# bitlayer-org/tap-stark

Measured on AMD Instinct MI355X. Metric: trace cells/sec (proofs/sec alongside), 2^20x64 BabyBear trace, higher is better.
Workload: dtype u32

## Files before the change

tap-stark_amd/csrc/kernels.hpp:

```cpp
#pragma once
#include <stdint.h>

#include "bb.hpp"
#include "context.hpp"
#include "ntt_plan.hpp"

namespace ts {

struct ColMat {
    uint32_t* d = nullptr;
    uint64_t height = 0;
    uint32_t width = 0;
    uint64_t col_stride = 0;
};

void launch_build_twiddles(Context& ctx, uint32_t* W, uint32_t* Winv, unsigned log_size);
void launch_build_plant_twiddles(Context& ctx, uint2* WP, uint2* WPinv, unsigned log_size);
void launch_build_shift_tables(Context& ctx, uint32_t* lo, uint32_t* hi, uint32_t n_hi,
                               uint32_t n_cosets, uint32_t shift_mont, unsigned log_N,
                               unsigned log_blowup, uint32_t scale_mont);
const uint32_t* coset_scale_table(Context& ctx, unsigned log_n, unsigned log_blowup, uint32_t shift);
void launch_transpose_bitrev(Context& ctx, const uint32_t* src, uint32_t* dst, unsigned log_n,
                             uint32_t w, uint64_t dst_col_stride, uint32_t src_width = 0);
bool launch_transpose_bitrev_r16(Context& ctx, const uint32_t* src, uint32_t* dst, unsigned log_n, uint32_t w,
                                 uint64_t dst_col_stride, uint32_t src_width = 0);
void launch_transpose_plain(Context& ctx, const uint32_t* src, uint32_t* dst, uint64_t n, uint32_t w,
                            uint64_t dst_col_stride);
void launch_transpose_to_row_major(Context& ctx, const uint32_t* src, uint64_t col_stride,
                                   uint32_t* dst, uint64_t h, uint32_t w);
void launch_transpose_unbitrev(Context& ctx, const uint32_t* src, uint64_t col_stride, uint32_t* dst,
                               unsigned log_h, uint32_t w);
void coset_lde(Context& ctx, uint32_t* evals, uint64_t in_col_stride, uint32_t ncols, unsigned log_n,
               unsigned log_blowup, uint32_t shift, uint32_t* out, uint64_t out_col_stride,
               uint32_t beta0 = 0, uint32_t n_beta = 0, bool first_round_done = false,
               uint32_t* evals2 = nullptr, uint32_t shift2 = 0, uint32_t gw = 0, bool stage_timers = true);

constexpr uint32_t LDE_NO_OWN = 0xffffffffu;
int lde_own_coset_used(unsigned log_n, unsigned log_blowup, uint32_t shift);

inline void ntt_require_shape(const NttPlan& p, uint32_t ncols, uint64_t stride_a, uint64_t stride_b, bool lde) {
    if (const char* why = ntt_plan_refusal(p, ncols, stride_a, stride_b, lde)) throw Error(TS_ERR_INVALID, why);
}
void launch_contig_inverse(Context& ctx, const NttPlan& p, uint32_t* data, uint64_t col_stride, uint32_t ncols,
                           bool first_round_done = false, uint32_t* data2 = nullptr, uint32_t gw = 0xffffffffu);
void launch_contig_forward(Context& ctx, const NttPlan& p, uint32_t* data, uint64_t col_stride, uint32_t ncols,
                           uint32_t n_blocks, uint32_t gw = 0xffffffffu, uint32_t own_a = LDE_NO_OWN,
                           uint32_t own_b = LDE_NO_OWN);

void dft_columns(Context& ctx, uint32_t* cols, uint64_t col_stride, uint32_t ncols, unsigned log_n, bool inverse,
                 uint32_t shift);
void dft_batch(Context& ctx, const uint32_t* in, uint32_t* out, unsigned log_n, uint32_t w, bool inverse,
               uint32_t shift);
void coset_lde_batch(Context& ctx, const uint32_t* in, uint32_t* out, unsigned log_n, uint32_t w, unsigned added_bits,
                     uint32_t shift, bool bit_reversed);
void launch_bit_reverse_rows(Context& ctx, const uint32_t* src, uint32_t* dst, unsigned log_h, uint32_t w);

constexpr int MAX_BATCH_MATS = 64;
struct LeafMats {
    const uint32_t* d[MAX_BATCH_MATS];
    uint64_t col_stride[MAX_BATCH_MATS];
    uint32_t width[MAX_BATCH_MATS];
    uint8_t row_shift[MAX_BATCH_MATS];
    uint32_t n_mats;
    uint32_t total_width;
    const uint32_t* const* cols;
};
void launch_leaf_hash(Context& ctx, const LeafMats& mats, uint64_t height, uint32_t* digests);
void launch_leaf_hash_ef_pairs(Context& ctx, const uint32_t* vec, uint64_t n_rows, uint32_t* digests);
struct DevChallenger;
bool launch_merkle_levels(Context& ctx, uint32_t* tree, unsigned log_leaves,
                          DevChallenger* ch = nullptr, uint32_t* root_out = nullptr,
                          Ef* beta_out = nullptr);
void launch_merkle_tree_from(Context& ctx, uint32_t* tree, unsigned log_leaves, unsigned first_level,
                             DevChallenger* ch, uint32_t* root_out, Ef* beta_out);
bool leaf_tree_enabled(unsigned log_leaves);
void launch_commit_tree(Context& ctx, const LeafMats& mats, unsigned log_leaves, uint32_t* tree,
                        uint32_t* root_out = nullptr);
void launch_shard_top(Context& ctx, const uint32_t* subroots, uint32_t G, uint32_t* top,
                      DevChallenger* ch, uint32_t* root_out, Ef* beta_out);
void launch_merkle_one_level(Context& ctx, const uint32_t* children, uint32_t* parents,
                             uint64_t n_parents);
void launch_merkle_inject(Context& ctx, uint32_t* nodes, const uint32_t* inj, uint64_t n);
inline uint64_t merkle_level_offset(unsigned log_leaves, unsigned level) {
    uint64_t off = 0;
    for (unsigned l = 0; l < level; l++) off += (uint64_t)1 << (log_leaves - l);
    return off;
}
inline uint64_t merkle_total_digests(unsigned log_leaves) { return ((uint64_t)2 << log_leaves) - 1; }

struct AirProgram;
const uint32_t* selector_table(Context& ctx, unsigned log_n, unsigned log_qd, uint32_t shift);
constexpr int MAX_QUOTIENT_CHUNKS = 64;
struct QuotOut {
    uint32_t* chunk[MAX_QUOTIENT_CHUNKS];
};
constexpr uint32_t MAX_SIDE_MATS = 2;
struct SideLdes {
    uint32_t n = 0;
    const ColMat* m[MAX_SIDE_MATS] = {nullptr, nullptr};
};
void launch_quotient(Context& ctx, const AirProgram& air, const ColMat& trace_lde, unsigned log_n,
                     unsigned log_qd, const uint32_t* d_consts_mont, const uint32_t* d_alpha_pows_mont,
                     const QuotOut& out, uint64_t row_begin = 0, uint64_t row_end = 0,
                     uint32_t shift = GENERATOR, const SideLdes& side = SideLdes());
void launch_chunk_mix(Context& ctx, uint32_t* const* d_chunk_ptrs, uint32_t qd, uint64_t rows, uint64_t col_stride,
                      const uint32_t* d_mix_mont);

struct SideRows {
    uint32_t n = 0;
    const uint32_t* d[MAX_SIDE_MATS] = {nullptr, nullptr};
    uint32_t width[MAX_SIDE_MATS] = {0, 0};
};
void launch_check_constraints(Context& ctx, const AirProgram& air, const uint32_t* trace_row_major,
                              uint64_t n, const uint32_t* d_consts_mont,
                              unsigned long long* d_violation, const SideRows& side = SideRows());

void launch_bary_weights(Context& ctx, unsigned log_n, const Ef* points_mont, uint32_t n_points,
                         Ef* out, uint32_t coset_gen = 0);
struct BaryPending {
    DevBuf<uint32_t> partial[4];
    uint32_t* out[4] = {nullptr, nullptr, nullptr, nullptr};
    uint32_t n_blocks[4] = {0, 0, 0, 0}, n_words[4] = {0, 0, 0, 0};
    uint32_t n = 0, capacity = 2;
};
void launch_bary_dots(Context& ctx, const ColMat& m, unsigned log_n, const Ef* weights,
                      uint32_t n_points, Ef* out, BaryPending* pending = nullptr);
void launch_bary_finish(Context& ctx, BaryPending& pending);
struct ReduceArgs {
    Ef z_mont[2];
    Ef off_mont[2];
    Ef rys[2];
    uint32_t n_points;
    uint32_t accumulate;
};
void launch_reduce(Context& ctx, const ColMat& m, unsigned log_h, const uint32_t* d_alpha_pows_mont,
                   const ReduceArgs& args, Ef* ro);
struct FusedReduceArgs {
    Ef z_mont[2];
    Ef off_t[2];
    Ef k0, k1;
    const uint32_t* chunk_w;
    const uint32_t* chunk[MAX_QUOTIENT_CHUNKS];
    uint64_t chunk_stride;
    uint32_t n_chunks;
    uint64_t row0, rows;
};
struct LeadingMats {
    uint32_t n = 0;
    const ColMat* m[2] = {nullptr, nullptr};
    Ef off[2][2];
};
void launch_reduce_fused(Context& ctx, const ColMat& trace, unsigned log_h,
                         const uint32_t* d_alpha_pows_mont, const FusedReduceArgs& args, Ef* ro,
                         const LeadingMats& lead = LeadingMats());
void launch_reduce_low(Context& ctx, const ColMat& trace, unsigned log_n, const uint32_t* d_alpha_pows_mont,
                       const FusedReduceArgs& args, const Ef* weights, uint32_t* out);
void launch_ef_interleave(Context& ctx, const uint32_t* cols, uint64_t col_stride, uint64_t rows, Ef* out);

struct ClassJob {
    const uint32_t* d;
    uint64_t col_stride;
    uint32_t width;
    uint32_t has_next;
    const uint32_t* weights;
    Ef off[2];
};
struct ClassReduceArgs {
    Ef z_mont[2];
    Ef k0, k1;
};
void launch_reduce_class(Context& ctx, const ClassJob* d_jobs, uint32_t n_jobs, unsigned log_h,
                         const uint32_t* d_alpha_pows_mont, const ClassReduceArgs& args, Ef* ro);
struct BaryFinishJob {
    const uint32_t* partial;
    uint32_t* out;
    uint32_t n_blocks, n_words;
};
void launch_bary_finish_jobs(Context& ctx, const BaryFinishJob* d_jobs, const uint2* d_groups, uint32_t n_groups);

void launch_fri_fold(Context& ctx, const Ef* in, uint64_t h, Ef beta_canonical, Ef* out,
                     uint32_t* next_digests);
void launch_fri_fold_dev(Context& ctx, const Ef* in, uint64_t h, const Ef* d_beta, Ef* out,
                         uint32_t* next_digests, uint64_t h_global = 0, uint64_t row0 = 0);
struct FriRoundLaunch {
    const Ef* prev = nullptr;
    const Ef* d_beta_prev = nullptr;
    Ef* cur = nullptr;
    uint64_t h = 0;
    uint32_t* tree = nullptr;
    DevChallenger* ch = nullptr;
    uint32_t* root_out = nullptr;
    Ef* beta_out = nullptr;
    uint64_t h_global = 0, row0 = 0;
};
void launch_fri_commit_round(Context& ctx, const FriRoundLaunch& r);
constexpr int FRI_TAIL_LOG = 10;
constexpr uint32_t FRI_POW_NONE = 0xffffffffu;
void launch_fri_tail(Context& ctx, const Ef* in, uint32_t L0, uint32_t blowup, DevChallenger* ch,
                     Ef* tail_vecs, uint32_t* tail_trees, uint32_t* roots_out, Ef* betas_out,
                     Ef* final_out, uint32_t pow_bits = 0, uint32_t* pow_out = nullptr,
                     const Ef* beta_in = nullptr);
void launch_vec_add(Context& ctx, Ef* acc, const Ef* other, uint64_t n);
struct FriGatherDesc {
    const uint32_t* vec;
    const uint32_t* tree;
    uint32_t log_leaves;
    uint32_t shift;
    uint64_t out_vals;
    uint64_t out_path;
};
struct RowGatherJob {
    LeafMats mats;
    uint32_t shift;
    uint32_t pad;
    uint64_t out;
};
void launch_gather_queries(Context& ctx, const RowGatherJob* d_rows, uint32_t n_rows, uint32_t max_row_width,
                           const FriGatherDesc* d_descs, uint32_t n_descs, uint32_t max_log_leaves,
                           const uint32_t* d_indices, uint32_t n_idx, uint32_t* out);

double alu_ceiling(Context& ctx, int kind);
double bench_stage(Context& ctx, int stage, unsigned log_n, uint32_t width, unsigned log_blowup, uint32_t reps);

void launch_trace_fibonacci(Context& ctx, uint32_t* out, uint32_t a, uint32_t b, uint64_t n);
void launch_trace_synth_mul(Context& ctx, uint32_t* out, uint64_t n, uint32_t width, uint64_t seed);
void launch_trace_synth_ext(Context& ctx, uint32_t* out, uint64_t n, uint32_t width, uint64_t seed);

enum : uint8_t { COL_U32 = 0, COL_U16 = 1, COL_U8 = 2, COL_MONTY32 = 3, COL_MONTY31 = 4 };
struct IngestPlan {
    bool planar = false;
    uint64_t height = 0;
    uint32_t width = 0;
    uint64_t stride = 0;
    uint64_t bytes = 0;
    int uniform4 = -1;
    std::vector<uint64_t> table;
};
IngestPlan ingest_plan(const uint8_t* kinds, uint32_t n_kinds, bool planar, uint64_t row_stride, uint64_t height,
                       uint32_t width);
void launch_ingest(Context& ctx, const IngestPlan& plan, const uint8_t* src, uint32_t* out);
void launch_scale_words(Context& ctx, const uint32_t* in, uint32_t* out, uint64_t n, uint32_t mult);
uint32_t monty_ingest_factor(uint32_t kind);

}
```

tap-stark_amd/csrc/open.hip:

```cpp
#include "kernels.hpp"
#include "open_dev.hpp"

namespace ts {

constexpr int BW_ROWS = 4;

__global__ void __launch_bounds__(256)
k_bary_weights(unsigned log_n, const uint32_t* __restrict__ W, uint32_t gen_mont, Ef z0, Ef z1,
               uint32_t n_points, Ef* __restrict__ out) {
    const uint64_t n = 1ull << log_n;
    const uint64_t t0 = ((uint64_t)blockIdx.x * blockDim.x + threadIdx.x) * BW_ROWS;
    if (t0 >= n) return;
    Ef num[2 * BW_ROWS];
    uint32_t nrm[2 * BW_ROWS], pre[2 * BW_ROWS], xs[BW_ROWS];
    uint32_t run = R_MOD_P;
#pragma unroll
    for (int k = 0; k < BW_ROWS; k++) {
        const bool ok = t0 + k < n;
        uint32_t x = ok ? mont_mul(gen_mont, root_bitrev(W, log_n, t0 + k)) : R_MOD_P;
        xs[k] = x;
#pragma unroll
        for (int p = 0; p < 2; p++) {
            const Ef z = p == 0 ? z0 : z1;
            Ef u = Ef{{sub(z.c[0], x), z.c[1], z.c[2], z.c[3]}};
// ... 38 lines not shown
    constexpr int PER_THREAD = COLS * TR / 256;
    __shared__ uint32_t tile[16 * 257];
    __shared__ uint32_t wts[TR][NP * 4];
    __shared__ uint32_t red[4 * RS][COLS][NP * 4];
    const uint64_t n = 1ull << log_n;
    const uint32_t c0 = blockIdx.y * COLS;
    const uint32_t lane = threadIdx.x & 63, wv = threadIdx.x >> 6;
    const uint32_t cl = lane % COLS, rs = lane / COLS;
    const uint32_t sub = wv * RS + rs;
    const uint64_t row_begin = (uint64_t)blockIdx.x * rows_per_block;
    const uint64_t row_end = row_begin + rows_per_block < n ? row_begin + rows_per_block : n;
    uint64_t acc[NP * 4];
#pragma unroll
    for (int j = 0; j < NP * 4; j++) acc[j] = 0;
    for (uint64_t row0 = row_begin; row0 < row_end; row0 += TR) {
        uint32_t v[PER_THREAD];
#pragma unroll
        for (int k = 0; k < PER_THREAD; k++) {
            const uint32_t e = threadIdx.x + (uint32_t)k * 256;
            const uint32_t c = c0 + e / TR;
            const uint64_t t = row0 + e % TR;
            v[k] = (c < width && t < row_end) ? m[(uint64_t)c * col_stride + t] : 0u;
        }
        for (uint32_t e = threadIdx.x; e < (uint32_t)(TR * NP); e += 256) {
            const uint32_t p = e / TR, tt = e % TR;
            const uint64_t t = row0 + tt;
            Ef w = ef_zero();
            if (t < row_end) w = weights[(uint64_t)p * n + t];
            wts[tt][p * 4 + 0] = w.c[0];
            wts[tt][p * 4 + 1] = w.c[1];
            wts[tt][p * 4 + 2] = w.c[2];
            wts[tt][p * 4 + 3] = w.c[3];
        }
#pragma unroll
        for (int k = 0; k < PER_THREAD; k++) {
            const uint32_t e = threadIdx.x + (uint32_t)k * 256;
            const uint32_t t = e % TR;
            tile[(t & 15) * 257 + (t >> 4) * COLS + e / TR] = v[k];
        }
        __syncthreads();
#pragma unroll
        for (int rr = 0; rr < 16; rr++) {
            const uint32_t tt = sub * 16 + rr;
            const uint32_t x = tile[rr * 257 + sub * COLS + cl];
#pragma unroll
            for (int j = 0; j < NP * 4; j++) acc[j] = lazy_mac(acc[j], x, wts[tt][j]);
            if (rr & 1) {
#pragma unroll
                for (int j = 0; j < NP * 4; j++) acc[j] = lazy_fix(acc[j]);
            }
        }
        __syncthreads();
    }
#pragma unroll
    for (int j = 0; j < NP * 4; j++) red[sub][cl][j] = lazy_finish(acc[j]);
    __syncthreads();
    for (uint32_t idx = threadIdx.x; idx < (uint32_t)(COLS * NP * 4); idx += 256) {
        const uint32_t c = idx / (NP * 4), j = idx % (NP * 4);
        uint32_t sum = 0;
#pragma unroll
        for (int q = 0; q < 4 * RS; q++) sum = add(sum, red[q][c][j]);
        if (c0 + c < width)
            partial[((uint64_t)blockIdx.x * width + c0 + c) * (NP * 4) + j] = sum;
    }
}

template <int N>
struct BaryFinishArgs {
    BaryFinishJob j[N];
    uint32_t groups[N];
};
template <int N>
__global__ void __launch_bounds__(256)
k_bary_finish(BaryFinishArgs<N> a) {
    BaryFinishJob j = a.j[0];
    uint32_t group = blockIdx.x, first = 0;
#pragma unroll
    for (int k = 1; k < N; k++) {
        first += a.groups[k - 1];
        if (blockIdx.x >= first) {
            j = a.j[k];
            group = blockIdx.x - first;
        }
    }
    bary_finish_group(j.partial, j.out, j.n_blocks, j.n_words, group);
}

template <int N>
static void launch_bary_finish_n(Context& ctx, const char* name, const BaryPending& pend) {
    BaryFinishArgs<N> a{};
    uint32_t total = 0;
    for (uint32_t i = 0; i < pend.n; i++) {
        a.j[i] = BaryFinishJob{pend.partial[i].p, pend.out[i], pend.n_blocks[i], pend.n_words[i]};
        a.groups[i] = (pend.n_words[i] + 3) / 4;
        total += a.groups[i];
    }
    TS_LAUNCH_NAMED(ctx, name, k_bary_finish<N>, dim3(total), dim3(256), 0, a);
}

void launch_bary_finish(Context& ctx, BaryPending& pend) {
    if (pend.n == 0) return;
    if (pend.n == 4)
        launch_bary_finish_n<4>(ctx, "k_bary_finish<4>", pend);
    else if (pend.n == 3)
        launch_bary_finish_n<3>(ctx, "k_bary_finish<3>", pend);
    else
        launch_bary_finish_n<2>(ctx, "k_bary_finish<2>", pend);
    TS_HIP(hipGetLastError());
    for (uint32_t i = 0; i < pend.n; i++) pend.partial[i].reset();
    pend.n = 0;
}

void launch_bary_dots(Context& ctx, const ColMat& m, unsigned log_n, const Ef* weights,
                      uint32_t n_points, Ef* out, BaryPending* pending) {
    const uint64_t n = 1ull << log_n;
    const bool narrow = m.width <= 8;
    const uint32_t tr = narrow ? 512 : 64;
    uint32_t n_blocks = (uint32_t)((n + tr - 1) / tr);
    if (n_blocks > 2048) n_blocks = 2048;
    uint32_t rows_per_block = (uint32_t)(((n + n_blocks - 1) / n_blocks + tr - 1) / tr * tr);
    n_blocks = (uint32_t)((n + rows_per_block - 1) / rows_per_block);
    const uint32_t n_words = m.width * n_points * 4;
    DevBuf<uint32_t> partial(&ctx, (size_t)n_blocks * n_words);
    const uint32_t* md = m.d;
    if (narrow) {
        dim3 grid(n_blocks, (m.width + 7) / 8);
        if (n_points == 2)
            TS_LAUNCH(ctx, (k_bary_dots<2, 8>), grid, dim3(256), 0, md, m.col_stride, m.width, log_n,
                      weights, partial.p, rows_per_block);
        else
            TS_LAUNCH(ctx, (k_bary_dots<1, 8>), grid, dim3(256), 0, md, m.col_stride, m.width, log_n,
                      weights, partial.p, rows_per_block);
    } else {
        dim3 grid(n_blocks, (m.width + 63) / 64);
        if (n_points == 2)
            TS_LAUNCH(ctx, (k_bary_dots<2, 64>), grid, dim3(256), 0, md, m.col_stride, m.width, log_n,
                      weights, partial.p, rows_per_block);
        else
            TS_LAUNCH(ctx, (k_bary_dots<1, 64>), grid, dim3(256), 0, md, m.col_stride, m.width, log_n,
                      weights, partial.p, rows_per_block);
    }
    TS_HIP(hipGetLastError());
    BaryPending own;
    BaryPending& pend = pending ? *pending : own;
    if (pend.n == pend.capacity) launch_bary_finish(ctx, pend);
    pend.partial[pend.n] = std::move(partial);
    pend.out[pend.n] = reinterpret_cast<uint32_t*>(out);
    pend.n_blocks[pend.n] = n_blocks;
    pend.n_words[pend.n] = n_words;
    pend.n++;
    if (!pending) launch_bary_finish(ctx, pend);
}

template <int NP>
__global__ void __launch_bounds__(256)
k_reduce(const uint32_t* __restrict__ m, uint64_t col_stride, uint32_t width, unsigned log_h,
         const uint32_t* __restrict__ W, uint32_t gen_mont, const uint32_t* __restrict__ alpha_pows,
         ReduceArgs args, Ef* __restrict__ ro) {
    const uint64_t h = 1ull << log_h;
    const uint64_t X = (uint64_t)blockIdx.x * blockDim.x + threadIdx.x;
    if (X >= h) return;
    const Ef S = row_dot_alpha(m, col_stride, width, X, alpha_pows);
    const uint32_t x = mont_mul(gen_mont, root_bitrev(W, log_h, X));
    Ef inv_d[NP];
    inv_denoms<NP>(x, args.z_mont, inv_d);
    Ef acc = args.accumulate ? ro[X] : ef_zero();
#pragma unroll
    for (int p = 0; p < NP; p++) {
        Ef t = ef_mul(ef_sub(S, args.rys[p]), args.off_mont[p]);
        acc = ef_add(acc, ef_mul(t, inv_d[p]));
    }
    ro[X] = acc;
}

void launch_reduce(Context& ctx, const ColMat& m, unsigned log_h, const uint32_t* d_alpha_pows_mont,
                   const ReduceArgs& args, Ef* ro) {
    TS_REQUIRE(args.n_points >= 1 && args.n_points <= 2, TS_ERR_INVALID, "reduce: 1 or 2 points");
    ctx.ensure_twiddles(log_h == 0 ? 1 : log_h);
    const uint64_t h = 1ull << log_h;
    dim3 grid((unsigned)((h + 255) / 256));
    if (args.n_points == 2)
        TS_LAUNCH(ctx, k_reduce<2>, grid, dim3(256), 0, (const uint32_t*)m.d, m.col_stride, m.width,
                  log_h, (const uint32_t*)ctx.d_twiddle_fwd, to_mont(GENERATOR), d_alpha_pows_mont, args,
                  ro);
    else
        TS_LAUNCH(ctx, k_reduce<1>, grid, dim3(256), 0, (const uint32_t*)m.d, m.col_stride, m.width,
                  log_h, (const uint32_t*)ctx.d_twiddle_fwd, to_mont(GENERATOR), d_alpha_pows_mont, args,
                  ro);
    TS_HIP(hipGetLastError());
}

template <int EXTRA>
struct ExtraReduceArgs {
    struct {
        const uint32_t* d;
        uint64_t stride;
        uint32_t width;
        Ef off[2];
    } m[EXTRA ? EXTRA : 1];
};

template <int EXTRA, bool LOW>
__global__ void __launch_bounds__(256)
k_reduce_fused(const uint32_t* __restrict__ trace, uint64_t trace_stride, uint32_t width, unsigned log_h,
               const uint32_t* __restrict__ W, uint32_t gen_mont, const uint32_t* __restrict__ alpha_pows,
               FusedReduceArgs a, ExtraReduceArgs<EXTRA> e, const Ef* __restrict__ weights,
               uint32_t* __restrict__ out) {
    const uint64_t X = (uint64_t)blockIdx.x * blockDim.x + threadIdx.x;
    if (X >= a.rows) return;
    const Ef St = row_dot_alpha(trace, trace_stride, width, X, alpha_pows);
    Ef inv_d[2];
    if constexpr (!LOW) {
        const uint32_t x = mont_mul(gen_mont, root_bitrev(W, log_h, a.row0 + X));
        inv_denoms<2>(x, a.z_mont, inv_d);
    }
    uint64_t acc[4] = {0, 0, 0, 0};
    uint32_t c = 0;
    for (; c + 2 <= a.n_chunks; c += 2) {
        uint32_t v[8];
#pragma unroll
        for (int k = 0; k < 8; k++) v[k] = a.chunk[c + (k >> 2)][(uint64_t)(k & 3) * a.chunk_stride + X];
        const uint32_t* ap = a.chunk_w + 16 * c;
#pragma unroll
        for (int k = 0; k < 8; k++) {
#pragma unroll
            for (int j = 0; j < 4; j++) acc[j] = lazy_mac(acc[j], v[k], ap[4 * k + j]);
            if (k & 1) {
#pragma unroll
                for (int j = 0; j < 4; j++) acc[j] = lazy_fix(acc[j]);
            }
        }
    }
    for (; c < a.n_chunks; c++) row_dot_acc(acc, a.chunk[c], a.chunk_stride, 4, X, a.chunk_w + 16 * c);
    const Ef D{{lazy_finish(acc[0]), lazy_finish(acc[1]), lazy_finish(acc[2]), lazy_finish(acc[3])}};
    if constexpr (LOW) {
        const uint32_t nxi = neg(mont_mul(gen_mont, root_bitrev(W, log_h, X)));
        inv_d[0] = ef_mul_base(weights[X], nxi);
        inv_d[1] = ef_mul_base(weights[a.rows + X], nxi);
    }
    Ef g0 = ef_add(ef_mul(St, a.off_t[0]), D), g1 = ef_mul(St, a.off_t[1]);
#pragma unroll
    for (int i = 0; i < EXTRA; i++) {
        const Ef S = row_dot_alpha(e.m[i].d, e.m[i].stride, e.m[i].width, X, alpha_pows);
        g0 = ef_add(g0, ef_mul(S, e.m[i].off[0]));
        g1 = ef_add(g1, ef_mul(S, e.m[i].off[1]));
    }
    const Ef r = ef_add(ef_mul(ef_sub(g0, a.k0), inv_d[0]), ef_mul(ef_sub(g1, a.k1), inv_d[1]));
    if constexpr (LOW) {
#pragma unroll
        for (int k = 0; k < 4; k++) out[(uint64_t)k * a.rows + X] = r.c[k];
    } else {
        *reinterpret_cast<uint4*>(out + 4 * X) = make_uint4(r.c[0], r.c[1], r.c[2], r.c[3]);
    }
}

template <int EXTRA>
static void launch_reduce_fused_n(Context& ctx, const char* name, const ColMat& trace, unsigned log_h,
                                  const uint32_t* d_alpha_pows_mont, const FusedReduceArgs& a,
                                  const LeadingMats& lead, Ef* ro) {
    ExtraReduceArgs<EXTRA> e{};
    for (int i = 0; i < EXTRA; i++) {
        e.m[i].d = lead.m[i]->d;
        e.m[i].stride = lead.m[i]->col_stride;
        e.m[i].width = lead.m[i]->width;
        e.m[i].off[0] = lead.off[i][0];
        e.m[i].off[1] = lead.off[i][1];
    }
    TS_LAUNCH_NAMED(ctx, name, (k_reduce_fused<EXTRA, false>), dim3((unsigned)((a.rows + 255) / 256)), dim3(256), 0,
                    (const uint32_t*)trace.d, trace.col_stride, trace.width, log_h,
                    (const uint32_t*)ctx.d_twiddle_fwd, to_mont(GENERATOR), d_alpha_pows_mont, a, e,
                    (const Ef*)nullptr, reinterpret_cast<uint32_t*>(ro));
}

void launch_reduce_fused(Context& ctx, const ColMat& trace, unsigned log_h,
                         const uint32_t* d_alpha_pows_mont, const FusedReduceArgs& args, Ef* ro,
                         const LeadingMats& lead) {
    TS_REQUIRE(args.n_chunks <= (uint32_t)MAX_QUOTIENT_CHUNKS, TS_ERR_INVALID, "reduce_fused: too many chunks");
    ctx.ensure_twiddles(log_h == 0 ? 1 : log_h);
    FusedReduceArgs a = args;
    if (a.rows == 0) {
        a.row0 = 0;
        a.rows = 1ull << log_h;
    }
    TS_REQUIRE(a.row0 + a.rows <= (1ull << log_h), TS_ERR_INVALID, "reduce_fused: row range");
    TS_REQUIRE(lead.n <= 2, TS_ERR_INVARIANT, "reduce_fused: more than two leading matrices");
    for (uint32_t i = 0; i < lead.n; i++) {
        const ColMat* m = lead.m[i];
        TS_REQUIRE(m && m->d && a.row0 == 0 && m->height == a.rows && m->col_stride >= a.rows, TS_ERR_INVALID,
                   "reduce_fused: preprocessed or aux matrix shape");
    }
    if (lead.n == 2)
        launch_reduce_fused_n<2>(ctx, "k_reduce_fused_pre_aux", trace, log_h, d_alpha_pows_mont, a, lead, ro);
    else if (lead.n == 1)
        launch_reduce_fused_n<1>(ctx, "k_reduce_fused_pre", trace, log_h, d_alpha_pows_mont, a, lead, ro);
    else
        launch_reduce_fused_n<0>(ctx, "k_reduce_fused", trace, log_h, d_alpha_pows_mont, a, lead, ro);
    TS_HIP(hipGetLastError());
}

void launch_reduce_low(Context& ctx, const ColMat& trace, unsigned log_n, const uint32_t* d_alpha_pows_mont,
                       const FusedReduceArgs& args, const Ef* weights, uint32_t* out) {
    TS_REQUIRE(args.n_chunks <= (uint32_t)MAX_QUOTIENT_CHUNKS, TS_ERR_INVALID, "reduce_low: too many chunks");
    const uint64_t n = 1ull << log_n;
    TS_REQUIRE(args.row0 == 0 && trace.height >= n && trace.col_stride >= n && args.chunk_stride >= n, TS_ERR_INVALID,
               "reduce_low: the matrices must start with the low coset");
    ctx.ensure_twiddles(log_n == 0 ? 1 : log_n);
// ... 24 lines not shown
```

tap-stark_amd/csrc/prover.cpp:

```cpp
#include <string.h>

#include <algorithm>

#include "logup.hpp"
#include "prover_internal.hpp"

namespace ts {

void mmcs_commit(Context& ctx, PcsData& data) {
    const unsigned log_H = data.log_height;
    const uint64_t N = 1ull << log_H;
    bool uniform = true;
    for (auto& cm : data.ldes) uniform = uniform && cm.height == N;
    {
        StageTimer t(&ctx, "merkle_commit");
        data.tree = DevBuf<uint32_t>(&ctx, merkle_total_digests(log_H) * 8);
        std::vector<const uint32_t*> cols;
        struct Group { uint64_t height; size_t first; uint32_t total; };
        std::vector<Group> groups;
        for (unsigned lh = log_H + 1; lh-- > 0;) {
            const std::vector<const uint32_t*> gc = column_pointers(data.ldes, 1ull << lh);
            if (!gc.empty()) groups.push_back(Group{1ull << lh, cols.size(), (uint32_t)gc.size()});
            cols.insert(cols.end(), gc.begin(), gc.end());
        }
// ... 28 lines not shown
            DevBuf<uint32_t> inj(&ctx, 8 * (N / 2));
            size_t gi = 1;
            for (unsigned l = 1; l <= log_H; l++) {
                uint32_t* children = data.tree.p + 8 * merkle_level_offset(log_H, l - 1);
                uint32_t* parents = data.tree.p + 8 * merkle_level_offset(log_H, l);
                const uint64_t n_par = N >> l;
                launch_merkle_one_level(ctx, children, parents, n_par);
                if (gi < groups.size() && groups[gi].height == n_par) {
                    group_leaves(groups[gi], inj.p);
                    launch_merkle_inject(ctx, parents, inj.p, n_par);
                    gi++;
                }
            }
        }
        if (mail) {
            ctx.sync_point(mail, 32);
            memcpy(data.root, mail, 32);
        } else {
            d2h_sync(ctx, data.root, data.tree.p + 8 * (merkle_total_digests(log_H) - 1), 32);
        }
    }
}

std::unique_ptr<PcsData> TwoAdicFriPcs::commit(std::vector<DeviceMatrix>& evals,
                                               const std::vector<uint32_t>& domain_shifts, bool build_tree,
                                               bool keep_row_major) {
    auto data = std::make_unique<PcsData>();
    lde_stage(ctx_, fri_, evals, domain_shifts, 0, 0, true, *data, keep_row_major);
    if (build_tree) mmcs_commit(ctx_, *data);
    return data;
}

void check_side_matrix(const PcsData& data, const AirProgram& air, uint32_t i, uint64_t lde_height) {
    const bool aux = air.side_is_aux(i);
    const std::string what = aux ? "aux data" : "preprocessed key";
    TS_REQUIRE(data.ldes.size() == 1, TS_ERR_INVALID, what + ": exactly one committed matrix expected");
    TS_REQUIRE(i < air.n_side() && data.ldes[0].width == air.side_width(i), TS_ERR_INVALID,
               what + ": width differs from the AIR's " + (aux ? "aux" : "preprocessed") + " width");
    TS_REQUIRE(data.ldes[0].height == lde_height, TS_ERR_INVALID,
               what + ": LDE height is not the trace height << log_blowup");
}

std::vector<DeviceMatrix> TwoAdicFriPcs::quotient_chunks(const PcsData& trace_data,
                                                         const AirProgram& air,
                                                         const std::vector<uint32_t>& pis, Ef alpha,
                                                         const SideData& side) {
    TS_REQUIRE(trace_data.ldes.size() >= 1, TS_ERR_INVALID, "quotient: no trace matrix");
    TS_REQUIRE(trace_data.log_height >= fri_.log_blowup, TS_ERR_INVALID, "quotient: bad trace data");
    TS_REQUIRE(side.size() <= MAX_SIDE_MATS, TS_ERR_INVALID, "quotient: more than two committed side matrices");
    SideLdes ldes;
    for (const PcsData* d : side) {
        check_side_matrix(*d, air, ldes.n, trace_data.ldes[0].height);
        ldes.m[ldes.n++] = &d->ldes[0];
    }
    return quotient_chunks_slab(trace_data.ldes[0], trace_data.log_height - fri_.log_blowup, Slab{}, air,
                                pis, alpha, GENERATOR, ldes);
}

std::vector<DeviceMatrix> TwoAdicFriPcs::quotient_chunks_slab(const ColMat& lde_slab, unsigned log_n,
                                                              const Slab& slab, const AirProgram& air,
                                                              const std::vector<uint32_t>& pis, Ef alpha,
                                                              uint32_t domain_shift, const SideLdes& side) {
    StageTimer t(&ctx_, "compute quotient polynomial");
    TS_REQUIRE(side.n == air.n_side(), TS_ERR_INVALID,
               "quotient: an AIR needs the committed key of its preprocessed columns and the committed aux trace of "
               "its aux columns, and only such an AIR takes them");
    TS_REQUIRE(side.n == 0 || slab.rows == 0, TS_ERR_UNSUPPORTED, "quotient: preprocessed or aux columns on a slab");
    TS_REQUIRE(lde_slab.width == air.width, TS_ERR_INVALID, "quotient: trace width != AIR width");
    TS_REQUIRE(pis.size() == air.n_public_slots(), TS_ERR_INVALID, "quotient: wrong number of public values");
    const unsigned lqd = air.log_quotient_degree;
    TS_REQUIRE(lqd <= fri_.log_blowup, TS_ERR_INVARIANT,
               "quotient domain larger than the committed LDE (log_quotient_degree > log_blowup)");
    const uint64_t n = 1ull << log_n, qn = n << lqd;
    const uint32_t qd = 1u << lqd;
    const uint64_t slab_rows = slab.rows ? slab.rows : lde_slab.height;
    const uint64_t row_begin = std::min<uint64_t>(slab.row0, qn);
    const uint64_t row_end = std::min<uint64_t>(slab.row0 + slab_rows, qn);
    TS_REQUIRE(row_begin % n == 0 && row_end % n == 0, TS_ERR_INVALID, "quotient: slab must hold whole cosets");

    std::vector<uint32_t> consts = air_consts_mont(air, pis.data(), pis.size());
    consts.resize((consts.size() + 3) & ~(size_t)3, 0);
    const size_t n_consts = consts.size();
    const uint32_t K = air.n_constraints;
    const std::vector<uint32_t> pw = alpha_powers_mont(alpha, K);
    consts.resize(n_consts + std::max<size_t>(4 * (size_t)K, 4), 0);
    for (uint32_t i = 0; i < K; i++) memcpy(&consts[n_consts + 4 * (size_t)(K - 1 - i)], &pw[4 * (size_t)i], 16);
    DevBuf<uint32_t> d_consts(&ctx_, consts.size());
    h2d(ctx_, d_consts.p, consts.data(), consts.size() * 4);

    std::vector<DeviceMatrix> chunks(qd);
    QuotOut qo;
    memset(&qo, 0, sizeof qo);
    for (uint32_t c = 0; c < qd; c++) {
        chunks[c].buf = DevBuf<uint32_t>(&ctx_, 4 * n);
        chunks[c].height = n;
        chunks[c].width = 4;
        chunks[c].layout = DeviceMatrix::COL_MAJOR_BITREV;
        qo.chunk[c] = chunks[c].buf.p;
    }
    if (row_begin < row_end) {
        ColMat lde = lde_slab;
        lde.d = lde_slab.d - slab.row0;
        launch_quotient(ctx_, air, lde, log_n, lqd, d_consts.p, d_consts.p + n_consts, qo, row_begin, row_end,
                        domain_shift, side);
    }
    return chunks;
}

DevBuf<Ef> TwoAdicFriPcs::open_reduce(const PcsData& trace_data, const PcsData& quotient_data, Ef zeta,
                                      Ef alpha, std::vector<Ef>& opened_values, const SideData& side) {
    TS_REQUIRE(trace_data.log_height == quotient_data.log_height, TS_ERR_INVALID,
               "open: trace and quotient LDE heights differ");
    return open_reduce_slab(trace_data, quotient_data, trace_data.log_height, Slab{}, zeta, alpha,
                            opened_values, side);
}

DevBuf<Ef> TwoAdicFriPcs::open_reduce_slab(const PcsData& trace_data, const PcsData& quotient_data,
                                           unsigned log_N, const Slab& slab, Ef zeta, Ef alpha,
                                           std::vector<Ef>& opened_values, const SideData& side) {
    TS_REQUIRE(trace_data.ldes.size() == 1, TS_ERR_UNSUPPORTED, "open: one trace matrix expected");
    TS_REQUIRE(side.size() <= MAX_SIDE_MATS, TS_ERR_INVALID, "open: more than two rounds before the trace's");
    LeadingMats lead;
    for (const PcsData* d : side) {
        TS_REQUIRE(slab.rows == 0 && d->ldes.size() == 1 && d->ldes[0].height == trace_data.ldes[0].height,
                   TS_ERR_INVALID, "open: preprocessed or aux round shape");
        lead.m[lead.n++] = &d->ldes[0];
    }
    const unsigned log_n = log_N - fri_.log_blowup;
    const uint64_t n = 1ull << log_n;
    const uint64_t N = slab.rows ? slab.rows : 1ull << log_N;
    TS_REQUIRE(N >= n && trace_data.ldes[0].height == N, TS_ERR_INVALID, "open: slab shape");
    const uint32_t coset_gen =
        mul(GENERATOR, pow_canon(two_adic_generator(log_N), bitrev32(slab.beta0, fri_.log_blowup)));
    const ColMat& tr = trace_data.ldes[0];
    const uint32_t w = tr.width;
    const uint32_t qd = (uint32_t)quotient_data.ldes.size();
    for (auto& m : quotient_data.ldes)
        TS_REQUIRE(m.width == 4, TS_ERR_INVALID, "open: quotient chunks must have width 4");
    ctx_.ensure_twiddles(std::max(1u, log_N));
    const ColMat* two_point[3];
    uint32_t n_two = 0, max_w = 4;
    size_t chunks_at = 0;
    for (uint32_t i = 0; i < lead.n; i++) two_point[n_two++] = lead.m[i];
    two_point[n_two++] = &tr;
    for (uint32_t i = 0; i < n_two; i++) {
        chunks_at += 2 * (size_t)two_point[i]->width;
        max_w = std::max(max_w, two_point[i]->width);
    }

    const Ef zeta_next = efc_mul_base(zeta, two_adic_generator(log_n));
    const Ef pts_mont[2] = {ef_to_mont(zeta), ef_to_mont(zeta_next)};

    std::vector<Ef> raw(chunks_at + 4 * (size_t)qd);
    DevBuf<Ef> weights(&ctx_, 2 * n);
    {
        StageTimer t(&ctx_, "compute opened values with Lagrange interpolation");
        launch_bary_weights(ctx_, log_n, pts_mont, 2, weights.p, coset_gen);
        Ef* const mail = reinterpret_cast<Ef*>(ctx_.mailbox(4 * raw.size()));
        BaryPending pend;
        pend.capacity = n_two + 1;
        Ef* sums = mail;
        for (uint32_t i = 0; i < n_two; i++) {
            launch_bary_dots(ctx_, *two_point[i], log_n, weights.p, 2, sums, &pend);
            sums += 2 * (size_t)two_point[i]->width;
        }
        ColMat all;
        if (qd > 1 && columns_as_one_matrix(quotient_data.ldes, quotient_data.ldes[0].height, 0, all) &&
            all.width == 4 * qd) {
            launch_bary_dots(ctx_, all, log_n, weights.p, 1, sums, &pend);
        } else {
            for (uint32_t c = 0; c < qd; c++)
                launch_bary_dots(ctx_, quotient_data.ldes[c], log_n, weights.p, 1, sums + 4 * c, &pend);
        }
        launch_bary_finish(ctx_, pend);
        ctx_.sync_point(mail, raw.size() * sizeof(Ef));
        memcpy(raw.data(), mail, raw.size() * sizeof(Ef));
    }
    const Ef scale[2] = {bary_scale(zeta, coset_gen, n), bary_scale(zeta_next, coset_gen, n)};
    opened_values.assign(raw.size(), ef_zero());
    size_t at = 0;
    for (uint32_t i = 0; i < n_two; i++) {
        opened_from_raw(&raw[at], two_point[i]->width, 2, scale, &opened_values[at]);
        at += 2 * (size_t)two_point[i]->width;
    }
    opened_from_raw(&raw[at], 4 * qd, 1, scale, &opened_values[at]);

    StageTimer t(&ctx_, "reduce rows");
    const bool low = slab.rows == 0 && lead.n == 0 && reduce_low_wanted(w + 4 * qd);
    if (!low) weights.reset();
    DevBuf<Ef> ro(&ctx_, N);
    TS_REQUIRE(qd <= (uint32_t)MAX_QUOTIENT_CHUNKS, TS_ERR_UNSUPPORTED, "open: more than 64 quotient chunks");
    FusedReduceArgs a;
    memset(&a, 0, sizeof a);
    a.z_mont[0] = pts_mont[0];
    a.z_mont[1] = pts_mont[1];
    a.n_chunks = qd;
    a.chunk_stride = N;
    a.row0 = slab.row0;
    a.rows = N;
    AlphaLedger ledger(alpha, max_w);
    const Ef* ys = opened_values.data();
    for (uint32_t i = 0; i < n_two; i++) {
        const uint32_t mw = two_point[i]->width;
        Ef* const off = i < lead.n ? lead.off[i] : a.off_t;
        for (int p = 0; p < 2; p++, ys += mw) off[p] = ledger.visit(log_N, ys, mw, p).off;
    }
    std::vector<uint32_t> words = ledger.powers();
    const size_t n_apow = words.size();
    for (uint32_t c = 0; c < qd; c++, ys += 4) {
        TS_REQUIRE(quotient_data.ldes[c].col_stride == N, TS_ERR_INVALID, "open: chunk stride");
        a.chunk[c] = quotient_data.ldes[c].d;
        ledger.fold_weights(ledger.visit(log_N, ys, 4, 0).off, 4, words);
    }
    a.k0 = ledger.k(log_N, 0);
    a.k1 = ledger.k(log_N, 1);
    DevBuf<uint32_t> d_apow(&ctx_, words.size());
    h2d(ctx_, d_apow.p, words.data(), words.size() * 4);
    a.chunk_w = d_apow.p + n_apow;
    if (low) {
        DevBuf<uint32_t> ro_low(&ctx_, 4 * n), ro_cols(&ctx_, 4 * N);
        launch_reduce_low(ctx_, tr, log_n, d_apow.p, a, weights.p, ro_low.p);
        coset_lde(ctx_, ro_low.p, n, 4, log_n, fri_.log_blowup, 1, ro_cols.p, N, 0, 0, false, nullptr, 0, 0,
                  false);
        launch_ef_interleave(ctx_, ro_cols.p, N, N, ro.p);
    } else {
        launch_reduce_fused(ctx_, tr, log_N, d_apow.p, a, ro.p, lead);
    }
    return ro;
}

void TwoAdicFriPcs::open_batch(const PcsData& d, uint64_t index, std::vector<uint32_t>& rows,
                               std::vector<uint32_t>& path) {
    TS_REQUIRE(index < (1ull << d.log_height), TS_ERR_INVALID, "open_batch: index out of range");
    QueryGather qg(ctx_);
    const unsigned li = qg.add_indices({(uint32_t)index});
    const QueryGather::Slot o_rows = qg.add_rows(li, d.leaf_mats(), 0), o_path = qg.add_path(li, d.tree.p, d.log_height, 0);
    qg.run();
    rows.assign(qg.data(o_rows, 0), qg.data(o_rows, 0) + o_rows.words);
    path.assign(qg.data(o_path, 0), qg.data(o_path, 0) + o_path.words);
}

void TwoAdicFriPcs::fri_prove(std::vector<DevBuf<Ef>>& inputs, const std::vector<unsigned>& log_lens,
                              BfChallenger& challenger,
                              const std::vector<const PcsData*>& input_rounds,
                              std::vector<uint32_t>& pf, bool pass_through) {
    Context& ctx = ctx_;
    const FriConfig& fri = fri_;
    TS_REQUIRE(!inputs.empty() && inputs.size() == log_lens.size(), TS_ERR_INVALID, "FRI: no input");
    std::vector<const Ef*> in_ptr;
    for (auto& v : inputs) in_ptr.push_back(v.p);
    if (pass_through)
        TS_REQUIRE(input_rounds.empty() && log_lens.back() >= 1, TS_ERR_INVALID,
                   "FRI: pass-through input proof takes no committed batches");
    for (size_t k = 1; k < log_lens.size(); k++)
        TS_REQUIRE(log_lens[k] < log_lens[k - 1], TS_ERR_INVALID, "FRI: inputs must descend in height");
    const unsigned log_max_height = log_lens[0];
    TS_REQUIRE(log_lens.back() >= fri.log_blowup, TS_ERR_INVALID, "FRI: vector shorter than the blowup");
    for (const PcsData* d : input_rounds)
        TS_REQUIRE(d->log_height <= log_max_height, TS_ERR_INVALID,
                   "FRI: a committed batch is taller than every opened matrix");

    FriCommit st;
    Ef final_poly;
    {
        StageTimer t(&ctx, "FRI commit phase");
        fri_commit_begin(ctx, fri, log_max_height, challenger, st);
        fri_commit_rounds(ctx, fri, std::move(inputs[0]), 1ull << log_max_height, inputs, log_lens, 1, st);
        final_poly = fri_commit_finish(ctx, fri, challenger, st);
    }
    std::vector<FriRound>& rounds = st.rounds;
    const uint32_t R = (uint32_t)rounds.size();

    uint32_t pow_witness;
    {
        StageTimer t(&ctx, "grind for proof-of-work witness");
        pow_witness = fri_pow_witness(ctx, challenger, fri.proof_of_work_bits, st);
    }

    StageTimer tq(&ctx, "query phase");
    const uint32_t Q = fri.num_queries;
    std::vector<uint32_t> indices(Q);
    for (uint32_t q = 0; q < Q; q++) indices[q] = (uint32_t)challenger.sample_bits(log_max_height);

    const size_t n_in_rounds = input_rounds.size();
    QueryGather qg(ctx);
    const unsigned li = qg.add_indices(indices);
    std::vector<QueryGather::Slot> o_rows(n_in_rounds), o_path(n_in_rounds);
    for (size_t k = 0; k < n_in_rounds; k++) {
        const unsigned lh = input_rounds[k]->log_height;
        o_rows[k] = qg.add_rows(li, input_rounds[k]->leaf_mats(), log_max_height - lh);
        o_path[k] = qg.add_path(li, input_rounds[k]->tree.p, lh, log_max_height - lh);
    }
    std::vector<QueryGather::Opening> o_round(R);
    for (uint32_t r = 0; r < R; r++)
        o_round[r] = qg.add_round(li, rounds[r].vec, rounds[r].tree, rounds[r].log_leaves, r + 1);
    std::vector<QueryGather::Slot> o_pass(pass_through ? in_ptr.size() : 0);
    for (size_t k = 0; k < o_pass.size(); k++)
        o_pass[k] = qg.add_values(li, in_ptr[k], log_max_height - log_lens[k] + 1);
    qg.run();

    std::vector<ProofWriter::Batch> batches;
    for (const PcsData* d : input_rounds) batches.push_back({&d->ldes, d->log_height});
    std::vector<unsigned> round_depths;
    for (auto& r : rounds) round_depths.push_back(r.log_leaves);
    pf.reserve(pf.size() + 16 + 8 * (size_t)R +
               (size_t)Q * ProofWriter::words_per_query(batches, round_depths, o_pass.size()));
    ProofWriter pw(pf);
    pw.begin_rounds(R);
    for (uint32_t r = 0; r < R; r++) pw.commitment(rounds[r].root, 8);
    pw.begin_queries(Q);
    for (uint32_t q = 0; q < Q; q++) {
        pw.begin_input_proof((uint32_t)(pass_through ? in_ptr.size() : n_in_rounds));
        for (size_t k = 0; k < o_pass.size(); k++) {
            const uint32_t half = (indices[q] >> (log_max_height - log_lens[k])) & 1;
            pw.pass_through_value(log_lens[k], qg.data(o_pass[k], q) + 4 * half);
        }
        for (size_t k = 0; k < n_in_rounds; k++) {
            const unsigned lh = input_rounds[k]->log_height;
            pw.batch_opening(input_rounds[k]->ldes, qg.data(o_rows[k], q), lh, {{qg.data(o_path[k], q), lh}});
        }
        for (uint32_t r = 0; r < R; r++)
            pw.round_opening(qg.data(o_round[r].vals, q), rounds[r].log_leaves,
                             {{qg.data(o_round[r].path, q), rounds[r].log_leaves}});
    }
    pw.finish(final_poly, pow_witness);
}

std::vector<uint32_t> TwoAdicFriPcs::open(const std::vector<OpenRound>& rounds, BfChallenger& challenger,
                                          std::vector<Ef>& opened_values) {
    TS_REQUIRE(!rounds.empty(), TS_ERR_INVALID, "open: no rounds");
    const Ef alpha = challenger.sample();
    uint32_t max_w = 1;
    unsigned log_global_max = 0;
    for (auto& r : rounds) {
        TS_REQUIRE(r.data && r.points.size() == r.data->ldes.size(), TS_ERR_INVALID,
                   "open: one point list per committed matrix");
        for (auto& m : r.data->ldes) max_w = std::max(max_w, m.width);
        log_global_max = std::max(log_global_max, r.data->log_height);
    }
    ctx_.ensure_twiddles(std::max(1u, log_global_max));
    AlphaLedger ledger(alpha, max_w);
// ... 204 lines not shown
```

Before: 26.36 billion.

## Fuse barycentric weight computation with multi-matrix dot products in one kernel

Adds a kernel that computes the Lagrange barycentric weights for each row block into shared memory and immediately takes dot products against the trace and quotient-chunk matrices in the same launch. This avoids a separate weights kernel, writing and re-reading the weights array from global memory, and one launch per matrix. The weights buffer is now allocated and written only when the later low-reduce or lead matrices need it. In exchange, each block carries a larger shared-memory footprint and recomputes the inversions per block, and the lead matrices are still handled by the older path.

```diff
diff --git a/tap-stark_amd/csrc/kernels.hpp b/tap-stark_amd/csrc/kernels.hpp
--- a/tap-stark_amd/csrc/kernels.hpp
+++ b/tap-stark_amd/csrc/kernels.hpp
@@ -126,6 +126,14 @@
 void launch_bary_dots(Context& ctx, const ColMat& m, unsigned log_n, const Ef* weights,
                       uint32_t n_points, Ef* out, BaryPending* pending = nullptr);
 void launch_bary_finish(Context& ctx, BaryPending& pending);
+constexpr int BARY_LIST_MAX = 4;
+struct BaryListMat {
+    const ColMat* m;
+    uint32_t n_points;
+    Ef* out;
+};
+void launch_bary_dots_list(Context& ctx, const BaryListMat* mats, uint32_t n_mats, unsigned log_n,
+                           const Ef* points_mont, uint32_t coset_gen, Ef* weights_out, BaryPending& pending);
 struct ReduceArgs {
     Ef z_mont[2];
     Ef off_mont[2];
diff --git a/tap-stark_amd/csrc/open.hip b/tap-stark_amd/csrc/open.hip
--- a/tap-stark_amd/csrc/open.hip
+++ b/tap-stark_amd/csrc/open.hip
@@ -214,6 +214,182 @@
     if (!pending) launch_bary_finish(ctx, pend);
 }
 
+constexpr int BL_ROWS = 512;
+
+template <int NP, int COLS>
+__device__ __forceinline__ void bary_dots_group(const uint32_t* __restrict__ m, uint64_t col_stride, uint32_t width,
+                                                uint32_t c0, uint64_t row0, uint64_t row_end,
+                                                uint32_t (*wts)[BL_ROWS][4], uint32_t* tile,
+                                                uint32_t* __restrict__ partial, bool first) {
+    constexpr int RS = 64 / COLS;
+    constexpr int TR = 16 * 4 * RS;
+    constexpr int PER_THREAD = COLS * TR / 256;
+    static_assert(BL_ROWS % TR == 0 && 256 * NP * 4 <= 16 * 257, "image and tile shapes");
+    uint32_t tid = threadIdx.x;
+    asm volatile("" : "+v"(tid));
+    const uint32_t lane = tid & 63, wv = tid >> 6;
+    const uint32_t cl = lane % COLS, rs = lane / COLS;
+    const uint32_t sub = wv * RS + rs;
+    const uint64_t img_end = row0 + BL_ROWS < row_end ? row0 + BL_ROWS : row_end;
+    uint64_t acc[NP * 4];
+#pragma unroll
+    for (int j = 0; j < NP * 4; j++) acc[j] = 0;
+    for (uint64_t r = row0; r < img_end; r += TR) {
+        uint32_t v[PER_THREAD];
+#pragma unroll
+        for (int k = 0; k < PER_THREAD; k++) {
+            const uint32_t e = tid + (uint32_t)k * 256;
+            const uint32_t c = c0 + e / TR;
+            const uint64_t t = r + e % TR;
+            v[k] = (c < width && t < img_end) ? m[(uint64_t)c * col_stride + t] : 0u;
+        }
+#pragma unroll
+        for (int k = 0; k < PER_THREAD; k++) {
+            const uint32_t e = tid + (uint32_t)k * 256;
+            const uint32_t t = e % TR;
+            tile[(t & 15) * 257 + (t >> 4) * COLS + e / TR] = v[k];
+        }
+        __syncthreads();
+        const uint32_t tt0 = (uint32_t)(r - row0) + sub * 16;
+#pragma unroll 8
+        for (int rr = 0; rr < 16; rr++) {
+            const uint32_t x = tile[rr * 257 + sub * COLS + cl];
+#pragma unroll
+            for (int j = 0; j < NP * 4; j++) acc[j] = lazy_mac(acc[j], x, wts[j >> 2][tt0 + rr][j & 3]);
+            if (rr & 1) {
+#pragma unroll
+                for (int j = 0; j < NP * 4; j++) acc[j] = lazy_fix(acc[j]);
+            }
+        }
+        __syncthreads();
+    }
+    uint32_t* red = tile;
+#pragma unroll
+    for (int j = 0; j < NP * 4; j++) red[(sub * COLS + cl) * (NP * 4) + j] = lazy_finish(acc[j]);
+    __syncthreads();
+    for (uint32_t idx = tid; idx < (uint32_t)(COLS * NP * 4); idx += 256) {
+        const uint32_t c = idx / (NP * 4), j = idx % (NP * 4);
+        uint32_t sum = 0;
+#pragma unroll
+        for (int q = 0; q < 4 * RS; q++) sum = add(sum, red[(q * COLS + c) * (NP * 4) + j]);
+        if (c0 + c < width) {
+            uint32_t* dst = partial + ((uint64_t)blockIdx.x * width + c0 + c) * (NP * 4) + j;
+            *dst = first ? sum : add(sum, *dst);
+        }
+    }
+    __syncthreads();
+}
+
+struct BaryListArgs {
+    struct {
+        const uint32_t* d;
+        uint64_t stride;
+        uint32_t width;
+        uint32_t n_points;
+        uint32_t* partial;
+    } m[BARY_LIST_MAX];
+    uint32_t n;
+};
+
+__global__ void __launch_bounds__(256, 4)
+k_bary_dots_list(BaryListArgs a, unsigned log_n, const uint32_t* __restrict__ W, uint32_t gen_mont, Ef z0, Ef z1,
+                 Ef* __restrict__ weights_out, uint32_t rows_per_block) {
+    __shared__ uint32_t tile[16 * 257];
+    __shared__ uint32_t wts[2][BL_ROWS][4];
+    const uint64_t n = 1ull << log_n;
+    const uint64_t row_begin = (uint64_t)blockIdx.x * rows_per_block;
+    const uint64_t row_end = row_begin + rows_per_block < n ? row_begin + rows_per_block : n;
+    for (uint64_t row0 = row_begin; row0 < row_end; row0 += BL_ROWS) {
+        {
+            const uint64_t t0 = row0 + 2 * threadIdx.x;
+            Ef num[4];
+            uint32_t nrm[4], pre[4], xs[2];
+            uint32_t run = R_MOD_P;
+#pragma unroll
+            for (int k = 0; k < 2; k++) {
+                const bool ok = t0 + k < row_end;
+                const uint32_t x = ok ? mont_mul(gen_mont, root_bitrev(W, log_n, t0 + k)) : R_MOD_P;
+                xs[k] = x;
+#pragma unroll
+                for (int p = 0; p < 2; p++) {
+                    const Ef z = p == 0 ? z0 : z1;
+                    const Ef u = Ef{{sub(z.c[0], x), z.c[1], z.c[2], z.c[3]}};
+                    if (ok) {
+                        ef_inv_parts(u, num[2 * k + p], nrm[2 * k + p]);
+                    } else {
+                        num[2 * k + p] = ef_zero();
+                        nrm[2 * k + p] = R_MOD_P;
+                    }
+                    pre[2 * k + p] = run;
+                    run = mont_mul(run, nrm[2 * k + p]);
+                }
+            }
+            uint32_t inv = mont_inv(run);
+#pragma unroll
+            for (int j = 3; j >= 0; j--) {
+                const uint32_t ninv = mont_mul(inv, pre[j]);
+                inv = mont_mul(inv, nrm[j]);
+                const int k = j >> 1, p = j & 1;
+                const Ef wt = ef_mul_base(num[j], mont_mul(ninv, xs[k]));
+                uint32_t* l = wts[p][2 * threadIdx.x + k];
+                l[0] = wt.c[0];
+                l[1] = wt.c[1];
+                l[2] = wt.c[2];
+                l[3] = wt.c[3];
+                if (weights_out != nullptr && t0 + k < row_end) weights_out[(uint64_t)p * n + t0 + k] = wt;
+            }
+        }
+        __syncthreads();
+        const bool first = row0 == row_begin;
+        for (uint32_t i = 0; i < a.n; i++) {
+            const uint32_t* const d = a.m[i].d;
+            const uint64_t stride = a.m[i].stride;
+            const uint32_t width = a.m[i].width;
+            uint32_t* const partial = a.m[i].partial;
+            if (a.m[i].n_points == 1) {
+                for (uint32_t c0 = 0; c0 < width; c0 += 8)
+                    bary_dots_group<1, 8>(d, stride, width, c0, row0, row_end, wts, tile, partial, first);
+            } else {
+                for (uint32_t c0 = 0; c0 < width; c0 += 64)
+                    bary_dots_group<2, 64>(d, stride, width, c0, row0, row_end, wts, tile, partial, first);
+            }
+        }
+    }
+}
+
+void launch_bary_dots_list(Context& ctx, const BaryListMat* mats, uint32_t n_mats, unsigned log_n,
+                           const Ef* points_mont, uint32_t coset_gen, Ef* weights_out, BaryPending& pend) {
+    TS_REQUIRE(n_mats >= 1 && n_mats <= (uint32_t)BARY_LIST_MAX && pend.n == 0 && pend.capacity >= n_mats,
+               TS_ERR_INVARIANT, "bary_dots_list: one to four matrices, all of them pending afterwards");
+    ctx.ensure_twiddles(log_n == 0 ? 1 : log_n);
+    const uint64_t n = 1ull << log_n;
+    uint32_t n_blocks = (uint32_t)((n + BL_ROWS - 1) / BL_ROWS);
+    if (n_blocks > 2048) n_blocks = 2048;
+    const uint32_t rows_per_block = (uint32_t)(((n + n_blocks - 1) / n_blocks + BL_ROWS - 1) / BL_ROWS * BL_ROWS);
+    n_blocks = (uint32_t)((n + rows_per_block - 1) / rows_per_block);
+    BaryListArgs a{};
+    a.n = n_mats;
+    for (uint32_t i = 0; i < n_mats; i++) {
+        const ColMat& m = *mats[i].m;
+        TS_REQUIRE(m.d && m.width >= 1 && m.col_stride >= n && (mats[i].n_points == 1 || mats[i].n_points == 2),
+                   TS_ERR_INVALID, "bary_dots_list: matrix shape or point count");
+        const uint32_t n_words = m.width * mats[i].n_points * 4;
+        pend.partial[i] = DevBuf<uint32_t>(&ctx, (size_t)n_blocks * n_words);
+        pend.out[i] = reinterpret_cast<uint32_t*>(mats[i].out);
+        pend.n_blocks[i] = n_blocks;
+        pend.n_words[i] = n_words;
+        a.m[i].d = m.d;
+        a.m[i].stride = m.col_stride;
+        a.m[i].width = m.width;
+        a.m[i].n_points = mats[i].n_points;
+        a.m[i].partial = pend.partial[i].p;
+    }
+    pend.n = n_mats;
+    TS_LAUNCH(ctx, k_bary_dots_list, dim3(n_blocks), dim3(256), 0, a, log_n, (const uint32_t*)ctx.d_twiddle_fwd,
+              to_mont(coset_gen ? coset_gen : GENERATOR), points_mont[0], points_mont[1], weights_out, rows_per_block);
+    TS_HIP(hipGetLastError());
+}
+
 template <int NP>
 __global__ void __launch_bounds__(256)
 k_reduce(const uint32_t* __restrict__ m, uint64_t col_stride, uint32_t width, unsigned log_h,
diff --git a/tap-stark_amd/csrc/prover.cpp b/tap-stark_amd/csrc/prover.cpp
--- a/tap-stark_amd/csrc/prover.cpp
+++ b/tap-stark_amd/csrc/prover.cpp
@@ -204,27 +204,41 @@
     const Ef pts_mont[2] = {ef_to_mont(zeta), ef_to_mont(zeta_next)};
 
     std::vector<Ef> raw(chunks_at + 4 * (size_t)qd);
-    DevBuf<Ef> weights(&ctx_, 2 * n);
+    const bool low = slab.rows == 0 && lead.n == 0 && reduce_low_wanted(w + 4 * qd);
+    DevBuf<Ef> weights;
+    if (low || lead.n) weights = DevBuf<Ef>(&ctx_, 2 * n);
     {
         StageTimer t(&ctx_, "compute opened values with Lagrange interpolation");
-        launch_bary_weights(ctx_, log_n, pts_mont, 2, weights.p, coset_gen);
         Ef* const mail = reinterpret_cast<Ef*>(ctx_.mailbox(4 * raw.size()));
-        BaryPending pend;
-        pend.capacity = n_two + 1;
-        Ef* sums = mail;
-        for (uint32_t i = 0; i < n_two; i++) {
-            launch_bary_dots(ctx_, *two_point[i], log_n, weights.p, 2, sums, &pend);
-            sums += 2 * (size_t)two_point[i]->width;
-        }
+        std::vector<BaryListMat> list;
+        std::vector<ColMat> chunk_mats;
+        Ef* sums = mail + (chunks_at - 2 * (size_t)w);
+        list.push_back(BaryListMat{&tr, 2, sums});
+        sums += 2 * (size_t)w;
         ColMat all;
         if (qd > 1 && columns_as_one_matrix(quotient_data.ldes, quotient_data.ldes[0].height, 0, all) &&
-            all.width == 4 * qd) {
-            launch_bary_dots(ctx_, all, log_n, weights.p, 1, sums, &pend);
-        } else {
-            for (uint32_t c = 0; c < qd; c++)
-                launch_bary_dots(ctx_, quotient_data.ldes[c], log_n, weights.p, 1, sums + 4 * c, &pend);
-        }
-        launch_bary_finish(ctx_, pend);
+            all.width == 4 * qd)
+            chunk_mats.push_back(all);
+        else
+            chunk_mats.assign(quotient_data.ldes.begin(), quotient_data.ldes.end());
+        for (const ColMat& m : chunk_mats) {
+            list.push_back(BaryListMat{&m, 1, sums});
+            sums += m.width;
+        }
+        for (size_t at = 0; at < list.size(); at += BARY_LIST_MAX) {
+            const uint32_t cnt = (uint32_t)std::min<size_t>(BARY_LIST_MAX, list.size() - at);
+            BaryPending pend;
+            pend.capacity = BARY_LIST_MAX;
+            launch_bary_dots_list(ctx_, &list[at], cnt, log_n, pts_mont, coset_gen, at == 0 ? weights.p : nullptr, pend);
+            if (at == 0) {
+                Ef* lead_sums = mail;
+                for (uint32_t i = 0; i < lead.n; i++) {
+                    launch_bary_dots(ctx_, *lead.m[i], log_n, weights.p, 2, lead_sums, &pend);
+                    lead_sums += 2 * (size_t)lead.m[i]->width;
+                }
+            }
+            launch_bary_finish(ctx_, pend);
+        }
         ctx_.sync_point(mail, raw.size() * sizeof(Ef));
         memcpy(raw.data(), mail, raw.size() * sizeof(Ef));
     }
@@ -238,7 +252,6 @@
     opened_from_raw(&raw[at], 4 * qd, 1, scale, &opened_values[at]);
 
     StageTimer t(&ctx_, "reduce rows");
-    const bool low = slab.rows == 0 && lead.n == 0 && reduce_low_wanted(w + 4 * qd);
     if (!low) weights.reset();
     DevBuf<Ef> ro(&ctx_, N);
     TS_REQUIRE(qd <= (uint32_t)MAX_QUOTIENT_CHUNKS, TS_ERR_UNSUPPORTED, "open: more than 64 quotient chunks");
```

New measurement: 26.28 billion. About the same (-0.3%).
